# microsoft/gated-graph-neural-network-samples

Measured on AMD Instinct MI355X. Metric: node-state updates/sec on QM9-shaped graphs, h=100, 4 edge types, higher is better.
Workload: dtype f32

## Files before the change

### gated-graph-neural-network-samples_amd/csrc/ggnn_gru_fused.hip

```cpp
#include "ggnn_split.hpp"
#include "ggnn_gru_cells.hpp"
#include <type_traits>

#ifndef GGNN_COOP_DEPTH
#define GGNN_COOP_DEPTH 1
#endif
#ifndef GGNN_GRU_STAMPS
#define GGNN_GRU_STAMPS 0
#endif
#if GGNN_GRU_STAMPS
#define GGNN_TDBG(a) (a).tdbg
#else
#define GGNN_TDBG(a) ((unsigned long long*)nullptr)
#endif

#ifndef GGNN_GRU_ABLATE
#define GGNN_GRU_ABLATE 0
#endif
#if GGNN_GRU_ABLATE
#define GGNN_ABL(BIT) ((ablate & (BIT)) != 0)
#define GGNN_ABL_PARAM , int ablate
#define GGNN_ABL_ARG , gru_ablate_bits()
static int gru_ablate_bits() { static const int v = [] { const char* e = getenv("GGNN_GRU_DBG"); return e ? atoi(e) : 0; }(); return v; }
#else
#define GGNN_ABL(BIT) (false)
#define GGNN_ABL_PARAM
#define GGNN_ABL_ARG
#endif

namespace ggnn {

int gru_panel_supported(int D);
int gru_panel_pack_floats(int D, int nx);
int gru_panel_launch_cell(const GruCell& c, const GruFusedArgs& a, float* packed, hipStream_t st);
int gru_wide_launch_cell(const GruCell& c, const GruFusedArgs& a, float* packed, hipStream_t st);

int gru_split_launch_cell(const GruCell& c, const GruFusedArgs& a, float* packed, hipStream_t st);

#ifndef GGNN_GRU_TU_SPLIT
int gru_pack_floats(int D, int nx) {
    if (gru_panel_supported(D)) return gru_panel_pack_floats(D, nx);
    const bool sp = split_matrix_path();
    static_assert(ImgCfg<100, true>::IMG >= ImgCfg<100, true, kSplitF16x2>::IMG && ImgCfg<64, true>::IMG >= ImgCfg<64, true, kSplitF16x2>::IMG &&
                  ImgCfg<32, true>::IMG >= ImgCfg<32, true, kSplitF16x2>::IMG, "bf16x3 images are the larger ones");
    switch (D) {
        case 100: return 3 * (nx + 1) * (sp ? ImgCfg<100, true>::IMG : ImgCfg<100, false>::IMG);
        case 64: return 3 * (nx + 1) * (sp ? ImgCfg<64, true>::IMG : ImgCfg<64, false>::IMG);
        case 32: return 3 * (nx + 1) * (sp ? ImgCfg<32, true>::IMG : ImgCfg<32, false>::IMG);
        default: return 0;
    }
}
#endif

template <int D, bool SPLIT, int FMT = kSplitBf16x3>
__global__ void gru_pack_weights_kernel(const float* __restrict__ Wg, const float* __restrict__ Wc, int nx,
                                        float* __restrict__ out) {
    const int ci = blockIdx.y;
    float* img = out + (size_t)ci * ImgCfg<D, SPLIT, FMT>::IMG;
    if constexpr (SPLIT) gru_fwd_image_pack_split<D, FMT>(Wg, Wc, nx, ci, img, blockIdx.x * blockDim.x + threadIdx.x, gridDim.x * blockDim.x);
    else gru_fwd_image_pack<D>(Wg, Wc, nx, ci, img, blockIdx.x * blockDim.x + threadIdx.x, gridDim.x * blockDim.x);
}

template <int NX>
__host__ __device__ constexpr int gru_stage_image(int pos) {
    return (pos % 3) < 2 ? 2 * (pos / 3) + (pos % 3) : 2 * (NX + 1) + pos / 3;
}

template <int FMT>
__device__ __forceinline__ f32x4 sigmoid4_acc(f32x4 z, f32x4 b_scaled) {
    constexpr float k = -kLog2e * SplitFmt<FMT>::acc_scale;
    return rcp_4(exp2_4(z * k + b_scaled) + 1.0f);
}
template <int FMT>
__device__ __forceinline__ f32x4 tanh4_acc(f32x4 z, f32x4 b_scaled) {
    constexpr float k = 2.0f * kLog2e * SplitFmt<FMT>::acc_scale;
    return 1.0f - 2.0f * rcp_4(exp2_4(z * k + b_scaled) + 1.0f);
}

__device__ __forceinline__ float row_up16(float x) {
    const unsigned u = __float_as_uint(x);
    return __uint_as_float(__builtin_amdgcn_permlane16_swap(u, u, false, false)[1]);
}
__device__ __forceinline__ float row_up32(float x) {
// ... 34 lines not shown

template <int D, int NX, int NW, bool SAVE, bool GATHER, bool SPLIT, bool SAVEX = SAVE, int FORM = 0, int FMT = kSplitBf16x3,
          int TK = kTkRuntime, bool G4AVG = false>
__global__ __launch_bounds__(NW * 64, FORM == 1 ? 2 : 1) void ggnn_gru_fused_kernel(GruFusedArgs a, const float* __restrict__ packed GGNN_ABL_PARAM) {
    static_assert(SPLIT || FMT == kSplitBf16x3, "the f32-MFMA kernels have no operand format");
    using C = StageCfg<D>;
    using I = ImgCfg<D, SPLIT, FMT>;
    using SC = SplitCfg<D, FMT>;
    constexpr bool HALF = FORM != 0;
    constexpr bool DEEP = FORM == 2;
    constexpr int NSLOT = DEEP ? 3 : 2;
    static_assert(!HALF || SPLIT, "the half-stage forms are split-form kernels");
    static_assert(FORM != 1 || NW == 4, "form 1 is the four-wave kernel");
    static_assert(!G4AVG || GATHER, "G4AVG fixes the gather's parameters");
    auto dyn_tk = [&]() -> bool {
        if constexpr (TK == kTkRuntime) return a.tickets != nullptr;
        else return TK == kTkCounter;
    };
    constexpr int NT = C::NT, NC = C::NC, NR = C::NR;
    constexpr int NSTAGE = 3 * (NX + 1);
    constexpr int SLOT = HALF ? SC::HA : I::IMG;
    extern __shared__ __attribute__((aligned(16))) float lds_[];

    const int tid = threadIdx.x, lane = tid & 63;
    const int wave = __builtin_amdgcn_readfirstlane(tid >> 6);
    const int li = lane & 15, kq = lane >> 4;
    if (GGNN_TDBG(a) && tid == 0) {
        a.tdbg[4096 + blockIdx.x * 4 + 0] = __builtin_amdgcn_s_memtime();
        a.tdbg[4096 + blockIdx.x * 4 + 1] = __builtin_amdgcn_s_memrealtime();
    }

    const int wt_total = (a.V + 15) / 16;
    const int nb = gridDim.x;
    const int full_tk = wt_total / (NW * nb) * nb;
    const int rest = wt_total - full_tk * NW;
    const int tail_w = (rest + nb - 1) / nb;
    const int n_tk = full_tk + (tail_w ? (rest + tail_w - 1) / tail_w : 0);
    const bool coop_tail = !HALF && (tail_w == 1) && (NT <= NW);
    auto is_coop = [&](int t) -> bool { return coop_tail && t >= full_tk && t < n_tk; };
    auto tile_of = [&](int t) -> int {
        if (t < full_tk) return t * NW + wave;
        if (t >= n_tk) return -1;
        if (coop_tail) return full_tk * NW + (t - full_tk);
        const int tl = full_tk * NW + (t - full_tk) * tail_w + wave;
        return (wave < tail_w && tl < wt_total) ? tl : -1;
    };

    constexpr int BIAS_FLOATS = (4 * D + 4 + 63) / 64 * 64;
    float* bias_s = lds_;
    float* ring = lds_ + BIAS_FLOATS;
    int* tk_slot = reinterpret_cast<int*>(bias_s + 4 * D);
    constexpr int RHP = C::BN + 4;
    float* rh_x = ring + NSLOT * SLOT;
    for (int i = tid; i < 4 * D; i += NW * 64)
        bias_s[i] = i < 2 * D ? -kLog2e * a.bg[i] : (i < 3 * D ? 2.0f * kLog2e * a.bc[i - 2 * D] : a.bc[i - 3 * D]);
    const bool late = FORM == 1 || wave >= NW / 2;
    int tk = blockIdx.x, tk_next = blockIdx.x + nb;
    if (dyn_tk() && tid == 0) *tk_slot = nb + atomicAdd(a.tickets, 1);

    int cur = 0;
    auto image_src = [&](int image) -> const float* {
        const float* p = packed;
        asm volatile("" : "+s"(p));
        return p + (size_t)image * I::IMG;
    };
    auto dma = [&](const float* src, float* dst) {
        if constexpr (SPLIT) dma_image_asm<I::IMG_BYTES, NW>(src, dst, wave, lane);
        else dma_image<I::IMG_BYTES, NW>(src, dst, wave, lane);
    };
    auto publish = [&]() { if constexpr (SPLIT) dma_wait(); __syncthreads(); };
    auto dma_ha = [&](const float* src, float* dst) { dma_kib_asm<SC::HA_BYTES / 1024, NW>(src, dst, wave, lane); };
    auto dma_hb = [&](const float* src, float* dst) { dma_kib_asm<SC::HB_BYTES / 1024, NW>(src, dst, wave, lane); };
    constexpr int KA = SC::HA_BYTES / 1024, KB = SC::HB_BYTES / 1024;
    const int own_a = KA / NW + (wave < KA % NW ? 1 : 0), own_b = KB / NW + (wave < KB % NW ? 1 : 0);
    auto publish_deep = [&](int own) {
        switch (own) {
            case 0: asm volatile("s_waitcnt vmcnt(0) lgkmcnt(0)" ::: "memory"); break;
            case 1: asm volatile("s_waitcnt vmcnt(1) lgkmcnt(0)" ::: "memory"); break;
            case 2: asm volatile("s_waitcnt vmcnt(2) lgkmcnt(0)" ::: "memory"); break;
            case 3: asm volatile("s_waitcnt vmcnt(3) lgkmcnt(0)" ::: "memory"); break;
            case 4: asm volatile("s_waitcnt vmcnt(4) lgkmcnt(0)" ::: "memory"); break;
            case 5: asm volatile("s_waitcnt vmcnt(5) lgkmcnt(0)" ::: "memory"); break;
            case 6: asm volatile("s_waitcnt vmcnt(6) lgkmcnt(0)" ::: "memory"); break;
            case 7: asm volatile("s_waitcnt vmcnt(7) lgkmcnt(0)" ::: "memory"); break;
            case 8: asm volatile("s_waitcnt vmcnt(8) lgkmcnt(0)" ::: "memory"); break;
            case 9: asm volatile("s_waitcnt vmcnt(9) lgkmcnt(0)" ::: "memory"); break;
            default: asm volatile("s_waitcnt vmcnt(10) lgkmcnt(0)" ::: "memory"); break;
        }
        __builtin_amdgcn_s_barrier();
    };
    static_assert(!DEEP || (SC::HA_BYTES / 1024 + NW - 1) / NW <= 10, "publish_deep covers <= 10 pieces per wave");
    if constexpr (DEEP) {
        dma_ha(packed, ring);
        dma_hb(packed + SC::HA, ring + SLOT);
    } else if constexpr (HALF) dma_ha(packed, ring);
    else dma(packed, ring);

    constexpr int GSEG = NX - 1, GBUF = GSEG & 1;
    constexpr int KI = 4;
    constexpr int G_U = NX == 1 ? NSTAGE : 3 * (NX - 1);
    constexpr bool G_NEXT = (NX == 1);
    constexpr bool G_RCP = NX == 1 || (FORM != 0 && D != 32);
    int g_beg = 0, g_end = 0;
    int g_i[KI] = {0, 0, 0, 0};
    f32x4 g_n = {0.f, 0.f, 0.f, 0.f};
    float g_den = 1.f, g_rcp = 1.f;
    Frag<D> gt;

    auto g_ptrs = [&](int r, bool on) {
        const int b = ldi_b(a.g_row_ptr, (unsigned)r * 4u), e = ldi_b(a.g_row_ptr, (unsigned)r * 4u + 4u);
        g_beg = on ? b : 0; g_end = on ? e : 0;
        if constexpr (G4AVG) {
            g_n = ld4_b(a.g_nin, (unsigned)r * 16u);
        } else if (a.g_use_avg) {
            if (a.g_T == 4) {
                g_n = ld4_b(a.g_nin, (unsigned)r * 16u);
            } else {
                float deg = 0.f;
                for (int t = 0; t < a.g_T; ++t) deg += a.g_nin[(size_t)r * a.g_T + t];
                g_n = f32x4{deg, 0.f, 0.f, 0.f};
            }
        }
    };
    auto touch = [](auto v) { asm volatile("" :: "v"(v)); };
    auto g_index = [&](int part) {
        if (part != 2) {
            touch(g_beg); touch(g_end);
            g_den = (((g_n.x + g_n.y) + g_n.z) + g_n.w) + 1e-7f;
            if constexpr (G_RCP) g_rcp = 1.0f / g_den;
        }
        if (part != 1) {
#pragma unroll
            for (int j = 0; j < KI; ++j) {
                g_i[j] = 0;
                if (g_beg + j < g_end) g_i[j] = ldi_b(a.g_idx, (unsigned)(g_beg + j) * 4u);
            }
        }
    };
    auto g_rows0 = [&](Frag<D>& f, int part) {
        if (part != 2) { touch(g_i[0]); touch(g_i[1]); touch(g_i[2]); touch(g_i[3]); }
        if (part != 1) {
            load_frag<D>(f, a.g_H, g_i[0], kq);
            load_frag<D>(gt, a.g_H, g_i[1], kq);
        }
    };
    auto g_rows = [&](Frag<D>& f, int k, int part) {
        if (part != 2) { if (g_beg + k - 1 < g_end) frag_add<D>(f, gt); }
        if (part != 1) load_frag<D>(gt, a.g_H, g_i[k], kq);
// ... 83 lines not shown
                if constexpr (POS == (P_R1 + NSTAGE) % NSTAGE) g_rows(xf[GBUF], 2, part);
                if constexpr (POS == (P_R2 + NSTAGE) % NSTAGE) g_rows(xf[GBUF], 3, part);
            }
            if (part != 1) {
                if constexpr (POS == 3 * NX - 1) load_frag<D>(hf, a.h, rowc, kq);
                if constexpr (j == 2 && s + 1 < NX && !(GATHER && s + 1 == GSEG)) load_frag<D>(xf[(s + 1) & 1], a.x[s + 1], rowc, kq);
                if constexpr (POS == NSTAGE - 1 && !(GATHER && GSEG == 0)) load_frag<D>(xf[0], a.x[0], rown, kq);
            }
        };

#if GGNN_GRU_STAMPS
#define GGNN_T(CI, K) if (a.tdbg && blockIdx.x == 0 && lane == 0 && p < 4) a.tdbg[((p * NSTAGE + (CI)) * NW + wave) * 4 + (K)] = __builtin_amdgcn_s_memtime();
#define GGNN_T2(CI, K) if (a.tdbg && blockIdx.x == 0 && lane == 0 && p < 4) a.tdbg[2048 + ((p * NSTAGE + (CI)) * NW + wave) * 4 + (K)] = __builtin_amdgcn_s_memtime();
#else
#define GGNN_T(CI, K)
#define GGNN_T2(CI, K)
#endif
#define GGNN_COOP_STAGE(POS, ACC, FRAG)                                                                  \
        {                                                                                                \
            GGNN_T(POS, 0)                                                                               \
            if constexpr (GATHER && (POS) == G_U % NSTAGE) {                                             \
                if (active && (!G_NEXT || p > 0)) { g_finish(xf[GBUF]); if constexpr (SAVEX) { if (row < a.V && a.save_x) store_x(xf[GBUF], row); } } \
            }                                                                                            \
            if constexpr ((POS) + TWD < NSTAGE) {                                                        \
                if (wave < NT) load_tile_weights<D>(tw[((POS) + TWD) % (TWD + 1)],                       \
                                                    packed + (size_t)gru_stage_image<NX>((POS) + TWD) * I::IMG, li, kq, wave); \
            }                                                                                            \
            prefetch(std::integral_constant<int, (POS)>{});                                              \
            if constexpr ((POS) == 3 * NX) {    \
                if (wave < NT && wave * 16 + 4 * kq < D) hv_pre = ld4_b(a.h, ((unsigned)rowc * D + wave * 16 + 4 * kq) * 4u); \
            }                                                                                            \
            GGNN_T(POS, 1)                                                                               \
            if (active && wave < NT && !GGNN_ABL(1)) {                                                   \
                if (C::TAILPACK3 && (POS) == NSTAGE - 1 && wave == NT - 1) {                             \
                     \
                    f32x4 t_;                                                                            \
                    tile_mma_regs<D, true>(t_, FRAG, tw[(POS) % (TWD + 1)]);                             \
                    ACC[0] = ACC[0] + t_;                                                                \
                } else tile_mma_regs<D, ((POS) < 3)>(ACC[0], FRAG, tw[(POS) % (TWD + 1)]);               \
            }                                                                                            \
            GGNN_T(POS, 2)                                                                               \
            if constexpr ((POS) == NSTAGE - 1) __syncthreads();    \
            GGNN_T(POS, 3)                                                                               \
        }
#define GGNN_HALF_STAGE(POS, ACC, FRAG)                                                                  \
        {                                                                                                \
            constexpr int npos_ = (POS) + 1;                                                             \
            const bool more_ = (npos_ < NSTAGE) || tk_next < n_dma;                                      \
            const float* csrc_ = image_src(gru_stage_image<NX>(POS));                     \
            const float* nsrc_ = image_src(gru_stage_image<NX>(npos_ < NSTAGE ? npos_ : 0)); \
            constexpr int ntl_ = ((C::TAILPACK && (POS) % 3 == 1) ||                                     \
                                  (C::TAILPACK3 && (POS) % 3 == 2 && (POS) < 3 * NX)) ? NT - 1 : NT;     \
            const int nxt_ = cur + 1 < NSLOT ? cur + 1 : 0, nx2_ = nxt_ + 1 < NSLOT ? nxt_ + 1 : 0;      \
            GGNN_T(POS, 0)                                                                               \
            if constexpr (GATHER && (POS) == G_U % NSTAGE) {     \
                if (active && (!G_NEXT || p > 0)) { g_finish(xf[GBUF]); if constexpr (SAVEX) { if (row < a.V && a.save_x) store_x(xf[GBUF], row); } } \
            }                                                                                            \
            if constexpr ((POS) % 3 == 0 || (POS) == NSTAGE - 1) { if (active && !GGNN_ABL(16)) split_frag<D, FMT>(sf, FRAG); } \
                                                      \
            bool dma_a_ = false;                                                                         \
            if constexpr (DEEP) {                                                                        \
                if (late) {                                                                              \
                    prefetch(std::integral_constant<int, (POS)>{}, 1);                                   \
                    if (more_ && !GGNN_ABL(8)) { dma_ha(nsrc_, ring + nx2_ * SLOT); dma_a_ = true; }     \
                    prefetch(std::integral_constant<int, (POS)>{}, 2);                                   \
                }                                                                                        \
            } else {                                                                                     \
                if (!GGNN_ABL(8)) dma_hb(csrc_ + SC::HA, ring + nxt_ * SLOT);                            \
                prefetch(std::integral_constant<int, (POS)>{});                                          \
            }                                                                                            \
            GGNN_T(POS, 1)                                                                               \
            __builtin_amdgcn_sched_barrier(0);                                                           \
            if GGNN_ABL(32) __builtin_amdgcn_s_setprio(3);                                               \
            if (active && !GGNN_ABL(1))                                                                  \
                stage_mma_split_at<D, (ntl_ < SC::TA ? ntl_ : SC::TA), ((POS) < 3), 0, false, FMT>(ACC, sf, FRAG, ring + cur * SLOT, ring + cur * SLOT, li, kq); \
            if GGNN_ABL(32) __builtin_amdgcn_s_setprio(0);                                               \
            __builtin_amdgcn_sched_barrier(0);                                                           \
            GGNN_T(POS, 2)                                                                               \
            if constexpr (DEEP) {                                                                        \
                if (!late) {                                                                             \
                    prefetch(std::integral_constant<int, (POS)>{}, 1);                                   \
                    if (more_ && !GGNN_ABL(8)) { dma_ha(nsrc_, ring + nx2_ * SLOT); dma_a_ = true; }     \
                    prefetch(std::integral_constant<int, (POS)>{}, 2);                                   \
                }                                                                                        \
                publish_deep(dma_a_ ? own_a : 0);                                                        \
            } else publish();                                                                            \
            GGNN_T(POS, 3)                                                                               \
            cur = nxt_;                                                                                  \
                       \
            {                                                                                            \
                const int nb1_ = cur + 1 < NSLOT ? cur + 1 : 0, nb2_ = nb1_ + 1 < NSLOT ? nb1_ + 1 : 0;  \
                bool dma_b_ = false;                                                                     \
                if constexpr (DEEP) {                                                                    \
                    if (late && more_ && !GGNN_ABL(8)) { dma_hb(nsrc_ + SC::HA, ring + nb2_ * SLOT); dma_b_ = true; } \
                } else {                                                                                 \
                    if (more_ && !GGNN_ABL(8)) dma_ha(nsrc_, ring + nb1_ * SLOT);                        \
                }                                                                                        \
                __builtin_amdgcn_sched_barrier(0);                                                       \
                GGNN_T2(POS, 0)                                                                          \
                if GGNN_ABL(32) __builtin_amdgcn_s_setprio(3);                                           \
                if (active && !GGNN_ABL(1))                                                              \
                    stage_mma_split_at<D, ntl_, ((POS) < 3), SC::TA, false, FMT>(ACC, sf, FRAG, ring + cur * SLOT, ring + cur * SLOT, li, kq); \
                if GGNN_ABL(32) __builtin_amdgcn_s_setprio(0);                                           \
                __builtin_amdgcn_sched_barrier(0);                                                       \
                GGNN_T2(POS, 1)                                                                          \
                if constexpr (DEEP) {                                                                    \
                    if (!late && more_ && !GGNN_ABL(8)) { dma_hb(nsrc_ + SC::HA, ring + nb2_ * SLOT); dma_b_ = true; } \
                    GGNN_T2(POS, 2)                                                                      \
                    publish_deep(dma_b_ ? own_b : 0);                                                    \
                } else publish();                                                                        \
                GGNN_T2(POS, 3)                                                                          \
                cur = nb1_;                                                                              \
            }                                                                                            \
        }
#define GGNN_STAGE(POS, ACC, FRAG)                                                                       \
        if constexpr (HALF) GGNN_HALF_STAGE(POS, ACC, FRAG) else                                         \
        if constexpr (coop && COOP_REGS) GGNN_COOP_STAGE(POS, ACC, FRAG) else                            \
        {                                                                                                \
            constexpr int npos_ = (POS) + 1;                                                             \
            const bool more_ = (npos_ < NSTAGE) || tk_next < n_dma;                                      \
            const float* nsrc_ = image_src(gru_stage_image<NX>(npos_ < NSTAGE ? npos_ : 0)); \
            float* ndst_ = ring + (cur ^ 1) * I::IMG;                                                    \
            GGNN_T(POS, 0)                                                                               \
            if constexpr (GATHER && (POS) == G_U % NSTAGE) {     \
                if (active && (!G_NEXT || p > 0)) { g_finish(xf[GBUF]); if constexpr (SAVEX) { if (row < a.V && a.save_x) store_x(xf[GBUF], row); } } \
            }                                                                                            \
                                                            \
            if (late) {                                                                                  \
                prefetch(std::integral_constant<int, (POS)>{});                                          \
                if (more_ && !GGNN_ABL(8)) dma(nsrc_, ndst_);                             \
            }                                                                                            \
            GGNN_T(POS, 1)                                                                               \
            __builtin_amdgcn_sched_barrier(0);     \
                      \
             \
            constexpr int ntl_ = ((C::TAILPACK && (POS) % 3 == 1) ||                                     \
                                  (C::TAILPACK3 && (POS) % 3 == 2 && (POS) < 3 * NX)) ? NT - 1 : NT;     \
                        \
                     \
            if constexpr (SPLIT && ((POS) % 3 == 0 || (POS) == NSTAGE - 1)) { if (active && !GGNN_ABL(16)) split_frag<D, FMT>(sf, FRAG); } \
            if GGNN_ABL(32) __builtin_amdgcn_s_setprio(3);                                               \
            if (active && !GGNN_ABL(1)) {                                                                \
                const float* img_ = ring + cur * I::IMG;                                                 \
                if constexpr (!coop) {                                                                   \
                    if constexpr (SPLIT) stage_mma_split<D, ntl_, ((POS) < 3), false, FMT>(ACC, sf, FRAG, img_, li, kq); \
                    else stage_mma<D, NoHook, ntl_, ((POS) < 3)>(ACC, FRAG, img_, li, kq);               \
                } else if (C::TAILPACK3 && (POS) == NSTAGE - 1 && wave == NT - 1) {                      \
                    f32x4 t_;         \
                    if constexpr (SPLIT) stage_mma_one_split<D, true, FMT>(t_, sf, FRAG, img_, li, kq, wave); \
                    else stage_mma_one<D, true>(t_, FRAG, img_, li, kq, wave);                           \
                    ACC[0] = ACC[0] + t_;                                                                \
                } else if (wave < NT) {                                                                  \
                    if constexpr (SPLIT) stage_mma_one_split<D, ((POS) < 3), FMT>(ACC[0], sf, FRAG, img_, li, kq, wave); \
                    else stage_mma_one<D, ((POS) < 3)>(ACC[0], FRAG, img_, li, kq, wave);                \
                }                                                                                        \
// ... 138 lines not shown
                    if (kq == q) hrem = f32x4{h0, h1, h2, h3};
                }
            }
        }
        if (active && row < a.V && !GGNN_ABL(4)) {
#pragma unroll
            for (int nt = 0; nt < NT; ++nt) {
                const int col = nt * 16 + 4 * kq;
                if (col < D) {
                    f32x4 hv;
                    if (nt < NC) hv = hf.v[nt];
                    else hv = hrem;
                    f32x4 c;
                    if (a.act == GGNN_ACT_TANH) {
                        c = tanh4_acc<FMT>(acc_c[nt], ld4(bias_s + 2 * D + col));
                    } else {
                        c = acc_c[nt] * SplitFmt<FMT>::acc_scale + ld4(bias_s + 3 * D + col);
                        c.x = fmaxf(c.x, 0.f); c.y = fmaxf(c.y, 0.f); c.z = fmaxf(c.z, 0.f); c.w = fmaxf(c.w, 0.f);
                    }
                    const f32x4 u = acc_u[nt];
                    st4_b(a.h_out, ((unsigned)row * D + col) * 4u, u * hv + (1.0f - u) * c);
                    if constexpr (SAVE) { if (a.save_c) st4_b(a.save_c, ((unsigned)row * D + col) * 4u, c); }
                }
            }
        }
    };
    int p = 0;
    for (; tk < n_main; ++p) run_pass(std::false_type{}, p);
    if constexpr (!HALF) { for (; tk < n_tk; ++p) run_pass(std::true_type{}, p); }
    if (GGNN_TDBG(a) && tid == 0) {
        a.tdbg[4096 + blockIdx.x * 4 + 2] = __builtin_amdgcn_s_memtime();
        a.tdbg[4096 + blockIdx.x * 4 + 3] = __builtin_amdgcn_s_memrealtime();
    }
}

template <int D, int NX, int NW, bool SAVE, bool GATHER, bool SPLIT, bool SAVEX = SAVE, int FORM = 0, int FMT = kSplitBf16x3,
          int TK = kTkRuntime, bool G4AVG = false>
static int launch_gru_fused_m(const GruFusedArgs& a_in, float* packed, hipStream_t st) {
    using C = StageCfg<D>;
    using I = ImgCfg<D, SPLIT, FMT>;
    GruFusedArgs a = a_in;
#if GGNN_GRU_STAMPS
    { const char* e = getenv("GGNN_GRU_TPTR"); a.tdbg = e ? (unsigned long long*)strtoull(e, nullptr, 10) : nullptr; }
#endif
    if (a.Wg) {
        hipLaunchKernelGGL((gru_pack_weights_kernel<D, SPLIT, FMT>), dim3(8, 3 * (NX + 1)), dim3(256), 0, st, a.Wg, a.Wc, NX, packed);
        GGNN_CHECK_HIP(hipGetLastError());
    }
    if (a.h == nullptr) return GGNN_OK;
    if ((unsigned long long)a.V * D >= (1ULL << 30) || (a.g_H && (unsigned long long)a.V * a.g_T * D >= (1ULL << 30)))
        return fail(GGNN_E_UNSUPPORTED, "fused GRU indexes with 32-bit byte offsets: V*D (and V*T*D for the gathered rows) "
                                        "must be < 2^30 (V=%d, D=%d)", a.V, D);
    constexpr size_t bias_b = (size_t)((4 * D + 4 + 63) / 64 * 64) * sizeof(float);
    const size_t lds = FORM == 1 ? (size_t)2 * SplitCfg<D, FMT>::HA_BYTES + bias_b
                     : FORM == 2 ? (size_t)3 * SplitCfg<D, FMT>::HA_BYTES + bias_b
                                 : (size_t)2 * I::IMG_BYTES + bias_b + (size_t)16 * (C::BN + 4) * sizeof(float);
    const int wt_total = (a.V + 15) / 16;
    int nb = FORM == 1 ? 2 * num_cus() : num_cus();
    if (nb > wt_total) nb = wt_total;
    if (FORM == 0 && gru_coop_small() && wt_total > nb && wt_total <= 2 * nb && StageCfg<D>::NT <= NW) nb = wt_total;
    static std::atomic<unsigned long long> lds_ok{0};
    if (lds > 64 * 1024) GGNN_CHECK_HIP(allow_dynamic_lds(&ggnn_gru_fused_kernel<D, NX, NW, SAVE, GATHER, SPLIT, SAVEX, FORM, FMT, TK, G4AVG>, lds, lds_ok));
    hipLaunchKernelGGL((ggnn_gru_fused_kernel<D, NX, NW, SAVE, GATHER, SPLIT, SAVEX, FORM, FMT, TK, G4AVG>), dim3(nb), dim3(NW * 64), lds, st, a, (const float*)packed GGNN_ABL_ARG);
    GGNN_CHECK_HIP(hipGetLastError());
    return GGNN_OK;
}

#ifdef GGNN_GRU_TU_SPLIT
int gru_split_launch_cell(const GruCell& c, const GruFusedArgs& a, float* packed, hipStream_t st) {
#ifdef GGNN_PROBE_NX
#ifndef GGNN_PROBE_SAVE
#define GGNN_PROBE_SAVE true
#endif
#ifndef GGNN_PROBE_SAVEX
#define GGNN_PROBE_SAVEX GGNN_PROBE_SAVE
#endif
#ifndef GGNN_PROBE_FMT
#define GGNN_PROBE_FMT kSplitF16x2
#endif
#ifndef GGNN_PROBE_FORM
#define GGNN_PROBE_FORM 0
#endif
#ifndef GGNN_PROBE_NW
#define GGNN_PROBE_NW 8
#endif
#ifndef GGNN_PROBE_TK
#define GGNN_PROBE_TK kTkRuntime
#endif
#ifndef GGNN_PROBE_G4AVG
#define GGNN_PROBE_G4AVG false
#endif
    (void)c;
    return launch_gru_fused_m<100, GGNN_PROBE_NX, GGNN_PROBE_NW, GGNN_PROBE_SAVE, true, true, GGNN_PROBE_SAVEX, GGNN_PROBE_FORM, GGNN_PROBE_FMT,
                              GGNN_PROBE_TK, GGNN_PROBE_G4AVG>(a, packed, st);
#else
    switch (gru_cell_key(c)) {
#define GGNN_GRU_RING_LAUNCH(D, NX, NW, SAVE, GATHER, SAVEX, FORM, FMT)                                                        \
        case gru_cell_key(GGNN_GRU_RING_CELL(D, NX, NW, SAVE, GATHER, SAVEX, FORM, FMT)):                                     \
            return launch_gru_fused_m<D, NX, NW, SAVE, GATHER, true, SAVEX, FORM, FMT>(a, packed, st);
#define GGNN_GRU_HOT_LAUNCH(NX, NW, FORM, FMT, TK)                                                                           \
        case gru_cell_key(GGNN_GRU_HOT_CELL(NX, NW, FORM, FMT, TK)):                                                         \
            return launch_gru_fused_m<100, NX, NW, false, true, true, false, FORM, FMT, TK, true>(a, packed, st);
        GGNN_GRU_RING_TABLE(GGNN_GRU_RING_LAUNCH)
        GGNN_GRU_HOT_TABLE(GGNN_GRU_HOT_LAUNCH)
#undef GGNN_GRU_RING_LAUNCH
#undef GGNN_GRU_HOT_LAUNCH
        default: return fail(GGNN_E_UNSUPPORTED, "fused GRU: the selected cell is not in the split-form table (D=%d nx=%d form=%d)", c.D, c.NX, c.FORM);
// ... 163 lines not shown
```

### gated-graph-neural-network-samples_amd/csrc/ggnn_split.hpp

```cpp
#pragma once
#include "ggnn_stage.hpp"
#include <type_traits>

namespace ggnn {

typedef __attribute__((ext_vector_type(8))) __bf16 bf16x8;
typedef __attribute__((ext_vector_type(4))) unsigned u32x4;

constexpr int kSplitBf16x3 = 3, kSplitF16x2 = 2;
template <int FMT> struct SplitFmt;
template <> struct SplitFmt<kSplitBf16x3> {
    static constexpr int NP = 3;
    static constexpr float w_scale = 1.0f, rem_scale = 1.0f, acc_scale = 1.0f;
};
template <> struct SplitFmt<kSplitF16x2> {
    static constexpr int NP = 2;
    static constexpr float w_scale = 256.0f;
    static constexpr float rem_scale = 256.0f;
    static constexpr float acc_scale = 1.0f / 256.0f;
};
typedef __attribute__((ext_vector_type(8))) _Float16 f16x8;
typedef __attribute__((ext_vector_type(2))) _Float16 f16x2;
#ifndef GGNN_F16_SPLIT_ASM
#define GGNN_F16_SPLIT_ASM 1
#endif
#ifndef GGNN_F16_CLAMP
#define GGNN_F16_CLAMP 0
#endif

int gru_fwd_fmt();
inline int gru_launch_fmt(int fmt) { return fmt == kSplitF16x2 ? kSplitF16x2 : kSplitBf16x3; }

bool split_matrix_path();

template <int D, int FMT = kSplitBf16x3>
struct SplitCfg {
    using S = StageCfg<D>;
    static constexpr bool OK = (S::NC % 2 == 0) && S::NC > 0;
    static constexpr int NC2 = S::NC / 2;
    static constexpr int TA = (S::NT + 1) / 2;
    static constexpr int NP = SplitFmt<FMT>::NP;
    static constexpr int plane_bytes(int nth) { return NC2 * 4 * nth * 16 * 16; }
    static constexpr int main_bytes(int nth) { return NP * plane_bytes(nth); }
    static constexpr int rem_bytes(int nth) { return S::NR * 4 * nth * 16 * 4; }
    static constexpr int half_bytes(int nth) { return (main_bytes(nth) + rem_bytes(nth) + 1023) / 1024 * 1024; }
    static constexpr int HA_BYTES = half_bytes(TA);
    static constexpr int HB_BYTES = half_bytes(S::NT - TA);
    static constexpr int HA = HA_BYTES / 4;
    static constexpr int IMG_BYTES = (HA_BYTES + HB_BYTES + 8191) / 8192 * 8192;
    static constexpr int IMG = IMG_BYTES / 4;
    static constexpr int half_of(int nt) { return nt < TA ? 0 : 1; }
    static constexpr int nth_of(int nt) { return nt < TA ? TA : S::NT - TA; }
    static constexpr int tile_in_half(int nt) { return nt < TA ? nt : nt - TA; }
};

template <int D, bool SPLIT, int FMT = kSplitBf16x3>
struct ImgCfg {
    static constexpr int IMG_BYTES = SPLIT ? SplitCfg<D, FMT>::IMG_BYTES : StageCfg<D>::IMG_BYTES;
    static constexpr int IMG = IMG_BYTES / 4;
};

__device__ __forceinline__ float trunc_bf16_f(float x) { return __uint_as_float(__float_as_uint(x) & 0xffff0000u); }

template <int FMT = kSplitBf16x3>
__device__ __forceinline__ unsigned split_piece_bits(float x, int p) {
    if constexpr (FMT == kSplitF16x2) {
#if GGNN_F16_CLAMP
        const float xs = fminf(fmaxf(x * SplitFmt<FMT>::w_scale, -65504.0f), 65504.0f);
#else
        const float xs = x * SplitFmt<FMT>::w_scale;
#endif
        const _Float16 h16 = (_Float16)xs;
        if (p == 0) return (unsigned)__builtin_bit_cast(unsigned short, h16);
        return (unsigned)__builtin_bit_cast(unsigned short, (_Float16)(xs - (float)h16));
    }
    const float hi = trunc_bf16_f(x);
    if (p == 0) return __float_as_uint(hi) >> 16;
    const float r1 = x - hi, mid = trunc_bf16_f(r1);
    if (p == 1) return __float_as_uint(mid) >> 16;
    return __float_as_uint(r1 - mid) >> 16;
}

template <int D>
struct StageValue {
    const float* W; int r0, c0, ldw, c_alt;
    const float* W2; int r0_2, ldw2, c_alt2;
    __device__ __forceinline__ float operator()(int k, int n) const {
        constexpr int TC = D % 16;
        if (n < D) return W[(size_t)(r0 + k) * ldw + c0 + n];
        if (c_alt >= 0 && n < D + TC) return W[(size_t)(r0 + k) * ldw + c_alt + (n - D)];
        if (W2 && c_alt2 >= 0 && n >= D + TC && n < D + 2 * TC) return W2[(size_t)(r0_2 + k) * ldw2 + c_alt2 + (n - D - TC)];
        return 0.f;
    }
};

template <int D>
struct StageValueT {
    const float* W; int r0, c0, ldw;
    __device__ __forceinline__ float operator()(int k, int n) const { return n < D ? W[(size_t)(r0 + n) * ldw + c0 + k] : 0.f; }
};

template <int D, int FMT = kSplitBf16x3, class Value>
__device__ __forceinline__ void pack_split_image(const Value& value, float* __restrict__ img, int first, int stride) {
    using C = SplitCfg<D, FMT>;
    using S = StageCfg<D>;
    for (int i = first; i < C::IMG; i += stride) {
// ... 71 lines not shown
    const unsigned v0 = __float_as_uint(r0), v1 = __float_as_uint(r1);
    m = __builtin_amdgcn_perm(v1, v0, 0x07060302u);
    const float s0 = r0 - __uint_as_float(v0 & 0xffff0000u), s1 = r1 - __uint_as_float(v1 & 0xffff0000u);
    l = __builtin_amdgcn_perm(__float_as_uint(s1), __float_as_uint(s0), 0x07060302u);
}

template <int D, int FMT = kSplitBf16x3>
__device__ __forceinline__ void split_frag(SFrag<D>& s, const Frag<D>& f) {
#pragma unroll
    for (int c2 = 0; c2 < SplitCfg<D>::NC2; ++c2) {
        const f32x4 a = f.v[2 * c2], b = f.v[2 * c2 + 1];
        unsigned h[4], m[4], l[4];
        split_pair<FMT>(a.x, a.y, h[0], m[0], l[0]);
        split_pair<FMT>(a.z, a.w, h[1], m[1], l[1]);
        split_pair<FMT>(b.x, b.y, h[2], m[2], l[2]);
        split_pair<FMT>(b.z, b.w, h[3], m[3], l[3]);
        s.hi[c2] = u32x4{h[0], h[1], h[2], h[3]};
        s.mid[c2] = u32x4{m[0], m[1], m[2], m[3]};
        s.lo[c2] = u32x4{l[0], l[1], l[2], l[3]};
    }
}

__device__ __forceinline__ f32x4 mfma_f16(u32x4 w, u32x4 a, f32x4 c) {
    return __builtin_amdgcn_mfma_f32_16x16x32_f16(__builtin_bit_cast(f16x8, w), __builtin_bit_cast(f16x8, a), c, 0, 0, 0);
}
__device__ __forceinline__ f32x4 mfma_bf16(u32x4 w, u32x4 a, f32x4 c) {
    return __builtin_amdgcn_mfma_f32_16x16x32_bf16(__builtin_bit_cast(bf16x8, w), __builtin_bit_cast(bf16x8, a), c, 0, 0, 0);
}

template <bool FIRST, int FMT = kSplitBf16x3>
__device__ __forceinline__ f32x4 split_products(f32x4 acc, u32x4 wh, u32x4 wm, u32x4 wl, u32x4 ah, u32x4 am, u32x4 al) {
    f32x4 c = FIRST ? f32x4{0.f, 0.f, 0.f, 0.f} : acc;
    if constexpr (FMT == kSplitF16x2) {
        c = mfma_f16(wm, ah, c);
        c = mfma_f16(wh, am, c);
        c = mfma_f16(wh, ah, c);
        return c;
    }
    c = mfma_bf16(wl, ah, c);
    c = mfma_bf16(wm, am, c);
    c = mfma_bf16(wm, ah, c);
    c = mfma_bf16(wh, al, c);
    c = mfma_bf16(wh, am, c);
    c = mfma_bf16(wh, ah, c);
    return c;
}

#ifndef GGNN_SPLIT_PF
#define GGNN_SPLIT_PF 0
#endif
#ifndef GGNN_SPLIT_WH2
#define GGNN_SPLIT_WH2 0
#endif
template <int D, int NTILES = StageCfg<D>::NT, bool ZERO = false, int T0 = 0, bool REMAT = false, int FMT = kSplitBf16x3>
__device__ __forceinline__ void stage_mma_split_at(f32x4 (&acc)[StageCfg<D>::NT], const SFrag<D>& a, const Frag<D>& af,
                                                   const float* img, const float* img_b, int li, int kq) {
    using S = StageCfg<D>;
    using C = SplitCfg<D, FMT>;
    if constexpr (REMAT) asm volatile("" : "+v"(li), "+v"(kq));
    constexpr int NTW = NTILES - T0;
    constexpr int NU = C::NC2 * NTW;
    if constexpr (NU > 0) {
        const u32x4* base_a = reinterpret_cast<const u32x4*>(img) + kq * (C::TA * 16) + li;
        const u32x4* base_b = reinterpret_cast<const u32x4*>(img_b) + kq * ((S::NT - C::TA) * 16) + li;
        auto slot = [&](int u, int p) {
            const int nt = T0 + u % NTW, c2 = u / NTW;
            const int nth = C::nth_of(nt);
            const u32x4* b = C::half_of(nt) ? base_b : base_a;
            return b[p * (C::plane_bytes(nth) / 16) + c2 * 4 * nth * 16 + C::tile_in_half(nt) * 16];
        };
      if constexpr (FMT == kSplitF16x2) {
        u32x4 wh = slot(0, 0), wm = slot(0, 1), nh = wh, nm = wm;
#pragma unroll
        for (int u = 0; u < NU; ++u) {
            const int c2 = u / NTW, nt = T0 + u % NTW;
            const bool more = u + 1 < NU;
            f32x4 c = (ZERO && c2 == 0) ? f32x4{0.f, 0.f, 0.f, 0.f} : acc[nt];
            if (more) { nm = slot(u + 1, 1); nh = slot(u + 1, 0); }
            __builtin_amdgcn_sched_barrier(0);
            c = mfma_f16(wm, a.hi[c2], c);
            c = mfma_f16(wh, a.mid[c2], c);
            c = mfma_f16(wh, a.hi[c2], c);
            __builtin_amdgcn_sched_barrier(0);
            wm = nm; wh = nh;
            acc[nt] = c;
        }
      } else {
        u32x4 wh = slot(0, 0), wm = slot(0, 1), wl = slot(0, 2);
#if GGNN_SPLIT_WH2
        u32x4 wh_n = wh;
#endif
#if GGNN_SPLIT_PF
        u32x4 nh = wh, nm = wm, nl = wl;
#pragma unroll
        for (int u = 0; u < NU; ++u) {
            const int c2 = u / NTW, nt = T0 + u % NTW;
            const bool more = u + 1 < NU;
            f32x4 c = (ZERO && c2 == 0) ? f32x4{0.f, 0.f, 0.f, 0.f} : acc[nt];
            if (more) { nl = slot(u + 1, 2); nm = slot(u + 1, 1); nh = slot(u + 1, 0); }
            __builtin_amdgcn_sched_barrier(0);
            c = mfma_bf16(wl, a.hi[c2], c);
            c = mfma_bf16(wm, a.mid[c2], c);
            c = mfma_bf16(wm, a.hi[c2], c);
            c = mfma_bf16(wh, a.lo[c2], c);
            c = mfma_bf16(wh, a.mid[c2], c);
            c = mfma_bf16(wh, a.hi[c2], c);
            __builtin_amdgcn_sched_barrier(0);
            wl = nl; wm = nm; wh = nh;
            acc[nt] = c;
        }
#else
#pragma unroll
        for (int u = 0; u < NU; ++u) {
            const int c2 = u / NTW, nt = T0 + u % NTW;
            const bool more = u + 1 < NU;
            f32x4 c = (ZERO && c2 == 0) ? f32x4{0.f, 0.f, 0.f, 0.f} : acc[nt];
#if GGNN_SPLIT_WH2
            if (more) wh_n = slot(u + 1, 0);
            __builtin_amdgcn_sched_barrier(0);
#endif
            c = mfma_bf16(wl, a.hi[c2], c);
            __builtin_amdgcn_sched_barrier(0);
            if (more) wl = slot(u + 1, 2);
            c = mfma_bf16(wm, a.mid[c2], c);
            c = mfma_bf16(wm, a.hi[c2], c);
            __builtin_amdgcn_sched_barrier(0);
            if (more) wm = slot(u + 1, 1);
            c = mfma_bf16(wh, a.lo[c2], c);
            c = mfma_bf16(wh, a.mid[c2], c);
            c = mfma_bf16(wh, a.hi[c2], c);
            __builtin_amdgcn_sched_barrier(0);
#if GGNN_SPLIT_WH2
            wh = wh_n;
#else
            if (more) wh = slot(u + 1, 0);
#endif
            acc[nt] = c;
        }
#endif
      }
    }
    if constexpr (S::NR > 0 && NTW > 0) {
        constexpr int NRM = S::NR * NTW;
        auto rw = [&](int i) {
            const int nt = T0 + i % NTW, q = i / NTW;
            const int nth = C::nth_of(nt);
            const float* b = C::half_of(nt) ? img_b : img;
            return b[C::main_bytes(nth) / 4 + (q * 4 + kq) * nth * 16 + li + C::tile_in_half(nt) * 16];
        };
        float w0 = rw(0), w1 = NRM > 1 ? rw(1) : 0.f;
#pragma unroll
        for (int i = 0; i < NRM; ++i) {
            const int q = i / NTW, nt = T0 + i % NTW;
            acc[nt] = __builtin_amdgcn_mfma_f32_16x16x4f32(w0, af.r[q], acc[nt], 0, 0, 0);
            __builtin_amdgcn_sched_barrier(0);
            w0 = w1;
            if (i + 2 < NRM) w1 = rw(i + 2);
        }
    }
}

template <int D, int NTILES = StageCfg<D>::NT, bool ZERO = false, bool REMAT = false, int FMT = kSplitBf16x3>
__device__ __forceinline__ void stage_mma_split(f32x4 (&acc)[StageCfg<D>::NT], const SFrag<D>& a, const Frag<D>& af,
                                                const float* img, int li, int kq) {
    stage_mma_split_at<D, NTILES, ZERO, 0, REMAT, FMT>(acc, a, af, img, img + SplitCfg<D, FMT>::HA, li, kq);
}

#define NC2_PLANE_SLOTS(NC2_, NTH_) ((NC2_) * 4 * (NTH_) * 16)
template <int D, bool ZERO, int FMT = kSplitBf16x3>
__device__ __forceinline__ void stage_mma_one_split(f32x4& acc, const SFrag<D>& a, const Frag<D>& af, const float* img, int li,
                                                    int kq, int tile) {
    using S = StageCfg<D>;
    using C = SplitCfg<D, FMT>;
    const bool hb = tile >= C::TA;
    const int nth = hb ? S::NT - C::TA : C::TA, til = hb ? tile - C::TA : tile;
    const float* him = hb ? img + C::HA : img;
    const int PL = NC2_PLANE_SLOTS(C::NC2, nth);
    const int CP = 4 * nth * 16;
    const u32x4* base = reinterpret_cast<const u32x4*>(him) + kq * nth * 16 + li + til * 16;
    f32x4 cin = acc;
    if constexpr (ZERO) cin = f32x4{0.f, 0.f, 0.f, 0.f};
    u32x4 w0 = base[0], w1 = base[PL], w2 = C::NP > 2 ? base[(C::NP - 1) * PL] : w1;
#pragma unroll
    for (int c2 = 0; c2 < C::NC2; ++c2) {
        const int cn = c2 + 1 < C::NC2 ? c2 + 1 : c2;
        const u32x4 n0 = base[cn * CP], n1 = base[PL + cn * CP], n2 = C::NP > 2 ? base[(C::NP - 1) * PL + cn * CP] : n1;
        cin = split_products<false, FMT>(cin, w0, w1, w2, a.hi[c2], a.mid[c2], a.lo[c2]);
        w0 = n0; w1 = n1; w2 = n2;
    }
#pragma unroll
    for (int q = 0; q < S::NR; ++q) {
        const float wr = him[C::NP * PL * 4 + (q * 4 + kq) * nth * 16 + li + til * 16];
        cin = __builtin_amdgcn_mfma_f32_16x16x4f32(wr, af.r[q], cin, 0, 0, 0);
    }
    acc = cin;
}

template <int BYTES, int NW>
__device__ __forceinline__ void dma_image(const float* src, float* dst, int wave, int lane) {
    constexpr int PER_WAVE = BYTES / (NW * 1024);
    static_assert(BYTES % (NW * 1024) == 0, "image must split into whole KiB per wave");
// ... 28 lines not shown
        const unsigned long long s = ((unsigned long long)hi << 32) | lo;
        const unsigned l = __builtin_amdgcn_readfirstlane(lbase + (unsigned)i0 * 1024u);
        constexpr int n = PER_WAVE;
        if (i0 + 3 < n)
            asm volatile("s_mov_b32 m0, %0\n\ts_nop 0\n\tglobal_load_lds_dwordx4 %1, %2\n\tglobal_load_lds_dwordx4 %1, %2 offset:1024\n\t"
                         "global_load_lds_dwordx4 %1, %2 offset:2048\n\tglobal_load_lds_dwordx4 %1, %2 offset:3072" :: "s"(l), "v"(voff), "s"(s) : "memory");
        else if (i0 + 2 < n)
            asm volatile("s_mov_b32 m0, %0\n\ts_nop 0\n\tglobal_load_lds_dwordx4 %1, %2\n\tglobal_load_lds_dwordx4 %1, %2 offset:1024\n\t"
                         "global_load_lds_dwordx4 %1, %2 offset:2048" :: "s"(l), "v"(voff), "s"(s) : "memory");
        else if (i0 + 1 < n)
            asm volatile("s_mov_b32 m0, %0\n\ts_nop 0\n\tglobal_load_lds_dwordx4 %1, %2\n\tglobal_load_lds_dwordx4 %1, %2 offset:1024"
                         :: "s"(l), "v"(voff), "s"(s) : "memory");
        else
            asm volatile("s_mov_b32 m0, %0\n\ts_nop 0\n\tglobal_load_lds_dwordx4 %1, %2" :: "s"(l), "v"(voff), "s"(s) : "memory");
    }
}
template <int KIB, int NW>
__device__ __forceinline__ void dma_kib_asm(const float* src, float* dst, int wave, int lane) {
    constexpr int Q = KIB / NW, R = KIB % NW;
    const unsigned voff = (unsigned)lane * 16u;
    const unsigned lds0 = (unsigned)(unsigned long)(lds_void*)dst;
    const unsigned long long src0 = reinterpret_cast<unsigned long long>(src);
    auto group = [&](unsigned byte_off, auto nc) {
        constexpr int n = decltype(nc)::value;
        const unsigned long long sb = src0 + byte_off;
        const unsigned lo = __builtin_amdgcn_readfirstlane((unsigned)sb);
        const unsigned hi = __builtin_amdgcn_readfirstlane((unsigned)(sb >> 32));
        const unsigned long long s = ((unsigned long long)hi << 32) | lo;
        const unsigned l = __builtin_amdgcn_readfirstlane(lds0 + byte_off);
        if constexpr (n == 4)
            asm volatile("s_mov_b32 m0, %0\n\ts_nop 0\n\tglobal_load_lds_dwordx4 %1, %2\n\tglobal_load_lds_dwordx4 %1, %2 offset:1024\n\t"
                         "global_load_lds_dwordx4 %1, %2 offset:2048\n\tglobal_load_lds_dwordx4 %1, %2 offset:3072" :: "s"(l), "v"(voff), "s"(s) : "memory");
        else if constexpr (n == 3)
            asm volatile("s_mov_b32 m0, %0\n\ts_nop 0\n\tglobal_load_lds_dwordx4 %1, %2\n\tglobal_load_lds_dwordx4 %1, %2 offset:1024\n\t"
                         "global_load_lds_dwordx4 %1, %2 offset:2048" :: "s"(l), "v"(voff), "s"(s) : "memory");
        else if constexpr (n == 2)
            asm volatile("s_mov_b32 m0, %0\n\ts_nop 0\n\tglobal_load_lds_dwordx4 %1, %2\n\tglobal_load_lds_dwordx4 %1, %2 offset:1024"
                         :: "s"(l), "v"(voff), "s"(s) : "memory");
        else
            asm volatile("s_mov_b32 m0, %0\n\ts_nop 0\n\tglobal_load_lds_dwordx4 %1, %2" :: "s"(l), "v"(voff), "s"(s) : "memory");
    };
#pragma unroll
    for (int i0 = 0; i0 < Q; i0 += 4) {
        const unsigned off = ((unsigned)wave * Q + (unsigned)i0) * 1024u;
        if (Q - i0 >= 4) group(off, std::integral_constant<int, 4>{});
        else if (Q - i0 == 3) group(off, std::integral_constant<int, 3>{});
        else if (Q - i0 == 2) group(off, std::integral_constant<int, 2>{});
        else group(off, std::integral_constant<int, 1>{});
    }
    if constexpr (R > 0) {
        if (wave < R) group(((unsigned)(NW * Q) + (unsigned)wave) * 1024u, std::integral_constant<int, 1>{});
    }
}
__device__ __forceinline__ void dma_wait() { __builtin_amdgcn_s_waitcnt(0x0F70); }

}
```

Measured before the change: 1.316 billion.

## Trim unused half-B tile columns from GRU weight DMA and add resident half-A option

For form-1 D=100 stages whose tail tile is unused, the half-B weight image is now streamed with a trimmed DMA that skips the last tile column, and the MMA indexing is made aware of the compacted LDS layout. This cuts global-to-LDS traffic and LDS footprint on those stages. An optional resident half-A slot, off by default, keeps the first stage's half-A in a third LDS slot so it is not refetched, at the cost of more LDS. The trimmed layout adds index complexity and risks misaddressing the remainder rows.

```diff
diff --git a/gated-graph-neural-network-samples_amd/csrc/ggnn_gru_fused.hip b/gated-graph-neural-network-samples_amd/csrc/ggnn_gru_fused.hip
--- a/gated-graph-neural-network-samples_amd/csrc/ggnn_gru_fused.hip
+++ b/gated-graph-neural-network-samples_amd/csrc/ggnn_gru_fused.hip
@@ -28,7 +28,17 @@
 #define GGNN_ABL_ARG
 #endif
 
+#ifndef GGNN_GRU_TRIM_HB
+#define GGNN_GRU_TRIM_HB 1
+#endif
+#ifndef GGNN_GRU_RESIDENT
+#define GGNN_GRU_RESIDENT 0
+#endif
+
 namespace ggnn {
+
+template <int D, int FORM, int FMT>
+constexpr bool gru_resident_half() { return GGNN_GRU_RESIDENT && FORM == 1 && D == 100 && FMT == kSplitF16x2; }
 
 int gru_panel_supported(int D);
 int gru_panel_pack_floats(int D, int nx);
@@ -169,6 +179,11 @@
     int* tk_slot = reinterpret_cast<int*>(bias_s + 4 * D);
     constexpr int RHP = C::BN + 4;
     float* rh_x = ring + NSLOT * SLOT;
+    constexpr bool TRIM = GGNN_GRU_TRIM_HB && FORM == 1 && D == 100 && SC::TRIM_OK;
+    constexpr bool RES = gru_resident_half<D, FORM, FMT>();
+    float* res_a = ring + NSLOT * SLOT;
+    unsigned trim_off = 0u;
+    if constexpr (TRIM) trim_off = SC::trim_lane_off((unsigned)lane);
     for (int i = tid; i < 4 * D; i += NW * 64)
         bias_s[i] = i < 2 * D ? -kLog2e * a.bg[i] : (i < 3 * D ? 2.0f * kLog2e * a.bc[i - 2 * D] : a.bc[i - 3 * D]);
     const bool late = FORM == 1 || wave >= NW / 2;
@@ -188,6 +203,9 @@
     auto publish = [&]() { if constexpr (SPLIT) dma_wait(); __syncthreads(); };
     auto dma_ha = [&](const float* src, float* dst) { dma_kib_asm<SC::HA_BYTES / 1024, NW>(src, dst, wave, lane); };
     auto dma_hb = [&](const float* src, float* dst) { dma_kib_asm<SC::HB_BYTES / 1024, NW>(src, dst, wave, lane); };
+    auto dma_hb_trim = [&](const float* src, float* dst) {
+        if constexpr (TRIM) dma_hb_trim_asm<D, FMT, NW>(src, dst, wave, lane, trim_off);
+    };
     constexpr int KA = SC::HA_BYTES / 1024, KB = SC::HB_BYTES / 1024;
     const int own_a = KA / NW + (wave < KA % NW ? 1 : 0), own_b = KB / NW + (wave < KB % NW ? 1 : 0);
     auto publish_deep = [&](int own) {
@@ -210,7 +228,7 @@
     if constexpr (DEEP) {
         dma_ha(packed, ring);
         dma_hb(packed + SC::HA, ring + SLOT);
-    } else if constexpr (HALF) dma_ha(packed, ring);
+    } else if constexpr (HALF) dma_ha(packed, RES ? res_a : ring);
     else dma(packed, ring);
 
     constexpr int GSEG = NX - 1, GBUF = GSEG & 1;
@@ -400,6 +418,11 @@
             constexpr int ntl_ = ((C::TAILPACK && (POS) % 3 == 1) ||                                     \
                                   (C::TAILPACK3 && (POS) % 3 == 2 && (POS) < 3 * NX)) ? NT - 1 : NT;     \
             const int nxt_ = cur + 1 < NSLOT ? cur + 1 : 0, nx2_ = nxt_ + 1 < NSLOT ? nxt_ + 1 : 0;      \
+             \
+            constexpr bool trim_ = TRIM && ntl_ == NT - 1 && ntl_ - SC::TA == SC::NTB - 1;               \
+            constexpr int nthb_ = trim_ ? SC::NTB - 1 : SC::NTB;                                         \
+             \
+            const float* ha_img_ = (RES && (POS) == 0) ? res_a : ring + cur * SLOT;                      \
             GGNN_T(POS, 0)                                                                               \
             if constexpr (GATHER && (POS) == G_U % NSTAGE) {     \
                 if (active && (!G_NEXT || p > 0)) { g_finish(xf[GBUF]); if constexpr (SAVEX) { if (row < a.V && a.save_x) store_x(xf[GBUF], row); } } \
@@ -414,14 +437,17 @@
                     prefetch(std::integral_constant<int, (POS)>{}, 2);                                   \
                 }                                                                                        \
             } else {                                                                                     \
-                if (!GGNN_ABL(8)) dma_hb(csrc_ + SC::HA, ring + nxt_ * SLOT);                            \
+                if (!GGNN_ABL(8)) {                                                                      \
+                    if constexpr (trim_) dma_hb_trim(csrc_ + SC::HA, ring + nxt_ * SLOT);                \
+                    else dma_hb(csrc_ + SC::HA, ring + nxt_ * SLOT);                                     \
+                }                                                                                        \
                 prefetch(std::integral_constant<int, (POS)>{});                                          \
             }                                                                                            \
             GGNN_T(POS, 1)                                                                               \
             __builtin_amdgcn_sched_barrier(0);                                                           \
             if GGNN_ABL(32) __builtin_amdgcn_s_setprio(3);                                               \
             if (active && !GGNN_ABL(1))                                                                  \
-                stage_mma_split_at<D, (ntl_ < SC::TA ? ntl_ : SC::TA), ((POS) < 3), 0, false, FMT>(ACC, sf, FRAG, ring + cur * SLOT, ring + cur * SLOT, li, kq); \
+                stage_mma_split_at<D, (ntl_ < SC::TA ? ntl_ : SC::TA), ((POS) < 3), 0, false, FMT>(ACC, sf, FRAG, ha_img_, ha_img_, li, kq); \
             if GGNN_ABL(32) __builtin_amdgcn_s_setprio(0);                                               \
             __builtin_amdgcn_sched_barrier(0);                                                           \
             GGNN_T(POS, 2)                                                                               \
@@ -441,14 +467,14 @@
                 bool dma_b_ = false;                                                                     \
                 if constexpr (DEEP) {                                                                    \
                     if (late && more_ && !GGNN_ABL(8)) { dma_hb(nsrc_ + SC::HA, ring + nb2_ * SLOT); dma_b_ = true; } \
-                } else {                                                                                 \
+                } else if constexpr (!(RES && npos_ == NSTAGE)) {    \
                     if (more_ && !GGNN_ABL(8)) dma_ha(nsrc_, ring + nb1_ * SLOT);                        \
                 }                                                                                        \
                 __builtin_amdgcn_sched_barrier(0);                                                       \
                 GGNN_T2(POS, 0)                                                                          \
                 if GGNN_ABL(32) __builtin_amdgcn_s_setprio(3);                                           \
                 if (active && !GGNN_ABL(1))                                                              \
-                    stage_mma_split_at<D, ntl_, ((POS) < 3), SC::TA, false, FMT>(ACC, sf, FRAG, ring + cur * SLOT, ring + cur * SLOT, li, kq); \
+                    stage_mma_split_at<D, ntl_, ((POS) < 3), SC::TA, false, FMT, nthb_>(ACC, sf, FRAG, ring + cur * SLOT, ring + cur * SLOT, li, kq); \
                 if GGNN_ABL(32) __builtin_amdgcn_s_setprio(0);                                           \
                 __builtin_amdgcn_sched_barrier(0);                                                       \
                 GGNN_T2(POS, 1)                                                                          \
@@ -693,7 +719,9 @@
         return fail(GGNN_E_UNSUPPORTED, "fused GRU indexes with 32-bit byte offsets: V*D (and V*T*D for the gathered rows) "
                                         "must be < 2^30 (V=%d, D=%d)", a.V, D);
     constexpr size_t bias_b = (size_t)((4 * D + 4 + 63) / 64 * 64) * sizeof(float);
-    const size_t lds = FORM == 1 ? (size_t)2 * SplitCfg<D, FMT>::HA_BYTES + bias_b
+    constexpr int form1_slots = gru_resident_half<D, FORM, FMT>() ? 3 : 2;
+    static_assert(FORM != 1 || 2 * ((size_t)form1_slots * SplitCfg<D, FMT>::HA_BYTES + bias_b) <= (size_t)160 * 1024, "two form-1 workgroups share a CU's LDS");
+    const size_t lds = FORM == 1 ? (size_t)form1_slots * SplitCfg<D, FMT>::HA_BYTES + bias_b
                      : FORM == 2 ? (size_t)3 * SplitCfg<D, FMT>::HA_BYTES + bias_b
                                  : (size_t)2 * I::IMG_BYTES + bias_b + (size_t)16 * (C::BN + 4) * sizeof(float);
     const int wt_total = (a.V + 15) / 16;
diff --git a/gated-graph-neural-network-samples_amd/csrc/ggnn_split.hpp b/gated-graph-neural-network-samples_amd/csrc/ggnn_split.hpp
--- a/gated-graph-neural-network-samples_amd/csrc/ggnn_split.hpp
+++ b/gated-graph-neural-network-samples_amd/csrc/ggnn_split.hpp
@@ -52,6 +52,15 @@
     static constexpr int half_of(int nt) { return nt < TA ? 0 : 1; }
     static constexpr int nth_of(int nt) { return nt < TA ? TA : S::NT - TA; }
     static constexpr int tile_in_half(int nt) { return nt < TA ? nt : nt - TA; }
+    static constexpr int NTB = S::NT - TA;
+    static constexpr int TRIM_ROW = (NTB - 1) * 256;
+    static constexpr bool TRIM_OK = OK && NTB >= 2 && (TRIM_ROW == 256 || TRIM_ROW == 512 || TRIM_ROW == 1024) &&
+                                    (NP * NC2 * 4 * TRIM_ROW) % 1024 == 0 && rem_bytes(NTB) <= 1024 &&
+                                    main_bytes(NTB) + 1024 <= HB_BYTES && main_bytes(NTB - 1) + 1024 <= HA_BYTES;
+    static constexpr int TRIM_MAIN_KIB = NP * NC2 * 4 * TRIM_ROW / 1024;
+    static __host__ __device__ constexpr unsigned trim_lane_off(unsigned lane) {
+        return lane * 16u / (unsigned)TRIM_ROW * (unsigned)(NTB * 256) + lane * 16u % (unsigned)TRIM_ROW;
+    }
 };
 
 template <int D, bool SPLIT, int FMT = kSplitBf16x3>
@@ -229,20 +238,23 @@
 #ifndef GGNN_SPLIT_WH2
 #define GGNN_SPLIT_WH2 0
 #endif
-template <int D, int NTILES = StageCfg<D>::NT, bool ZERO = false, int T0 = 0, bool REMAT = false, int FMT = kSplitBf16x3>
+template <int D, int NTILES = StageCfg<D>::NT, bool ZERO = false, int T0 = 0, bool REMAT = false, int FMT = kSplitBf16x3,
+          int NTHB = SplitCfg<D, FMT>::NTB>
 __device__ __forceinline__ void stage_mma_split_at(f32x4 (&acc)[StageCfg<D>::NT], const SFrag<D>& a, const Frag<D>& af,
                                                    const float* img, const float* img_b, int li, int kq) {
     using S = StageCfg<D>;
     using C = SplitCfg<D, FMT>;
     if constexpr (REMAT) asm volatile("" : "+v"(li), "+v"(kq));
+    static_assert(NTHB == C::NTB || (NTHB == C::NTB - 1 && NTILES <= C::TA + NTHB), "a trimmed half B holds the tiles the call walks");
+    auto nth_lds = [](int nt) constexpr { return nt < C::TA ? C::TA : NTHB; };
     constexpr int NTW = NTILES - T0;
     constexpr int NU = C::NC2 * NTW;
     if constexpr (NU > 0) {
         const u32x4* base_a = reinterpret_cast<const u32x4*>(img) + kq * (C::TA * 16) + li;
-        const u32x4* base_b = reinterpret_cast<const u32x4*>(img_b) + kq * ((S::NT - C::TA) * 16) + li;
+        const u32x4* base_b = reinterpret_cast<const u32x4*>(img_b) + kq * (NTHB * 16) + li;
         auto slot = [&](int u, int p) {
             const int nt = T0 + u % NTW, c2 = u / NTW;
-            const int nth = C::nth_of(nt);
+            const int nth = nth_lds(nt);
             const u32x4* b = C::half_of(nt) ? base_b : base_a;
             return b[p * (C::plane_bytes(nth) / 16) + c2 * 4 * nth * 16 + C::tile_in_half(nt) * 16];
         };
@@ -321,9 +333,8 @@
         constexpr int NRM = S::NR * NTW;
         auto rw = [&](int i) {
             const int nt = T0 + i % NTW, q = i / NTW;
-            const int nth = C::nth_of(nt);
             const float* b = C::half_of(nt) ? img_b : img;
-            return b[C::main_bytes(nth) / 4 + (q * 4 + kq) * nth * 16 + li + C::tile_in_half(nt) * 16];
+            return b[C::main_bytes(nth_lds(nt)) / 4 + (q * 4 + kq) * C::nth_of(nt) * 16 + li + C::tile_in_half(nt) * 16];
         };
         float w0 = rw(0), w1 = NRM > 1 ? rw(1) : 0.f;
 #pragma unroll
@@ -458,6 +469,33 @@
         if (wave < R) group(((unsigned)(NW * Q) + (unsigned)wave) * 1024u, std::integral_constant<int, 1>{});
     }
 }
+template <int D, int FMT, int NW>
+__device__ __forceinline__ void dma_hb_trim_asm(const float* src, float* dst, int wave, int lane, unsigned row_off) {
+    using C = SplitCfg<D, FMT>;
+    static_assert(C::TRIM_OK, "no trimmed half B at this size");
+    constexpr int KM = C::TRIM_MAIN_KIB, Q = KM / NW, R = KM % NW;
+    constexpr unsigned SRC_STEP = 1024u / C::TRIM_ROW * (C::NTB * 256u);
+    asm volatile("" : "+s"(wave));
+    const unsigned lds0 = (unsigned)(unsigned long)(lds_void*)dst;
+    const unsigned long long src0 = reinterpret_cast<unsigned long long>(src);
+    auto piece = [&](unsigned src_off, unsigned lds_off, unsigned voff) {
+        const unsigned long long sb = src0 + src_off;
+        const unsigned lo = __builtin_amdgcn_readfirstlane((unsigned)sb);
+        const unsigned hi = __builtin_amdgcn_readfirstlane((unsigned)(sb >> 32));
+        const unsigned long long s = ((unsigned long long)hi << 32) | lo;
+        const unsigned l = __builtin_amdgcn_readfirstlane(lds0 + lds_off);
+        asm volatile("s_mov_b32 m0, %0\n\ts_nop 0\n\tglobal_load_lds_dwordx4 %1, %2" :: "s"(l), "v"(voff), "s"(s) : "memory");
+    };
+#pragma unroll
+    for (int i = 0; i < Q; ++i) {
+        const unsigned k = (unsigned)wave * Q + (unsigned)i;
+        piece(k * SRC_STEP, k * 1024u, row_off);
+    }
+    if constexpr (R > 0) {
+        if (wave < R) piece((unsigned)(NW * Q + wave) * SRC_STEP, (unsigned)(NW * Q + wave) * 1024u, row_off);
+    }
+    if (wave == R % NW) piece((unsigned)C::main_bytes(C::NTB), (unsigned)C::main_bytes(C::NTB - 1), (unsigned)lane * 16u);
+}
 __device__ __forceinline__ void dma_wait() { __builtin_amdgcn_s_waitcnt(0x0F70); }
 
 }
```

Result: no change. 1.326 billion (median of 6 runs) (+0.8%).
